# cyrillefavreau/Sol-R

Measured on AMD Instinct MI355X. Metric: Mrays/s @1920x1080, 3-bounce Cornell, higher is better.
Workload: dtype f32; 1 GPU; cornell 1920x1080, 3 bounces + shadow rays, 75 boxes / 29 primitives, one GPU, whole frame; rays_per_frame=6518779, closest_hit_walks_rank0=3506171, lane_nodes=206382796, lane_prim_tests=37557299, wave_nodes=3396811, wave_prim_tests=626627, wave_walks=106204, cost_ordered_launch_rank0=True, frames_in_flight=3, setup_frames_before_warmup=48, frames_delivered=9105, order_free_nodes=43, short_ray_lists=1, gather=none (one GPU), strips=equal rows, parallelism=tile1

## Files before the change

include/solr_hip.h:

```cpp
#ifndef SOLR_HIP_H
#define SOLR_HIP_H

#include "solr_types.h"

#ifdef __cplusplus
extern "C" {
#endif


void initialize_scene(vec2i occupancyParameters, SceneInfo sceneInfo, int nbPrimitives, int nbLamps,
                      int nbMaterials);

void finalize_scene(vec2i occupancyParameters);

void reshape_scene(vec2i occupancyParameters, SceneInfo sceneInfo);

void h2d_scene(vec2i occupancyParameters, BoundingBox *boundingBoxes, int nbActiveBoxes, Primitive *primitives,
               int nbPrimitives, Lamp *lamps, int nbLamps);

void h2d_materials(vec2i occupancyParameters, Material *materials, int nbActiveMaterials);

void h2d_randoms(vec2i occupancyParameters, float *randoms);

void h2d_textures(vec2i occupancyParameters, int activeTextures, TextureInfo *textureInfos);
// ... 55 lines not shown
int solr_hip_build_tree(const Primitive *primitives, const unsigned char *emissive, int nbPrimitives,
                        const float minPos[3], const float maxPos[3], float viewDistance, BoundingBox *boxes,
                        int boxCapacity, int *order, int *nbBoxes, int *nbLamps);
const char *solr_hip_build_tree_message(void);

void *solr_hip_device_bitmap(void);
void *solr_hip_device_primitive_ids(void);
void *solr_hip_device_postprocessing(void);
void solr_hip_bind_device_bitmap(void *deviceBitmap);

void solr_hip_h2d_randoms_sized(const float *randoms, long count);

int solr_hip_d2h_image_async(void);
const BitmapBuffer *solr_hip_image_wait(int ticket);
void solr_hip_set_copy_route(int onTheFramesOwnStream);
int solr_hip_stream_next_image(int on);
int solr_hip_d2h_streamed_image(BitmapBuffer *image);
int solr_hip_d2h_streamed(BitmapBuffer *image, PrimitiveXYIdBuffer *primitivesXYIds);
int solr_hip_image_share(const char *name, int rank, int world);
void solr_hip_image_share_sealed(void);
void solr_hip_image_unshare(void);

void solr_hip_d2h_postprocessing(PostProcessingBuffer *hostBuffer);
void solr_hip_h2d_postprocessing(const PostProcessingBuffer *hostBuffer, const PrimitiveXYIdBuffer *ids);

void solr_hip_initialize(const SceneInfo *sceneInfo);
void solr_hip_reshape(const SceneInfo *sceneInfo);
void solr_hip_render(const SceneInfo *sceneInfo, const vec4i *objects, const PostProcessingInfo *postProcessingInfo,
                     const float origin[3], const float direction[3], const float angles[4]);
void solr_hip_d2h(const SceneInfo *sceneInfo, BitmapBuffer *bitmap, PrimitiveXYIdBuffer *primitivesXYIds);

void solr_hip_enable_timing(int enable);
double solr_hip_kernel_time(int *nbLaunches, int reset);
int solr_hip_timing_samples(float *kernelMs, float *intervalMs, int capacity);

void solr_hip_set_frames_in_flight(int n);
int solr_hip_get_frames_in_flight(void);
void *solr_hip_flight_stream(int flight);
int solr_hip_next_flight(void);
void solr_hip_set_flight_streams(void *const *streams, int n);

void solr_hip_set_tile_scheduling(int mode);
int solr_hip_tile_scheduling_active(void);
int solr_hip_split_tiles(void);

void solr_hip_enable_tile_clocks(int enable);
int solr_hip_tile_clocks(unsigned long long *clocks, int capacityTiles);

void solr_hip_render_counting(const SceneInfo *sceneInfo, const vec4i *objects,
                              const PostProcessingInfo *postProcessingInfo, const float origin[3],
                              const float direction[3], const float angles[4], unsigned long long counts[8]);

void solr_hip_set_variant(int variant);
void solr_hip_set_short_ray_lists(int mode);
int solr_hip_short_ray_lists(void);
int solr_hip_order_free_nodes(void);
int solr_hip_order_free_shadows(void);
int solr_hip_get_variant(void);

void solr_hip_set_movable(const unsigned char *flags, int nbPrimitives);
int solr_hip_rotate_primitives(const float center[3], const float cosAngles[3], const float sinAngles[3],
                               float viewDistance);
int solr_hip_device_rotations(void);
int solr_hip_read_nodes(int exact, float *rows, int capacityRows);
int solr_hip_read_primitives(float *rows, int capacityRows);

void solr_hip_memory_usage(unsigned long long bytes[4]);

#ifdef __cplusplus
}
#endif
#endif
```

sol-r_amd/csrc/engine.h:

```cpp
#ifndef SOLR_ENGINE_H
#define SOLR_ENGINE_H

#include <hip/hip_runtime.h>

#include <atomic>
#include <chrono>
#include <cstdio>
#include <cstdlib>
#include <cstring>
#include <string>
#include <vector>

#include "../../include/solr_hip.h"
#include "renderer.h"
#include "lists_device.h"

namespace solreng
{
struct HostProfile
{
    const bool on = getenv("SOLR_HIP_HOST_PROFILE") != nullptr;
    struct Entry
    {
        const char *name;
// ... 63 lines not shown
struct DeviceBuffer
{
    void *ptr = nullptr;
    size_t bytes = 0;
};

const int MAX_FLIGHTS = 4;
struct SharedRing
{
    std::atomic<long> done[64][MAX_FLIGHTS + 2];
    std::atomic<long> consumed;
    long frameBytes, imageStride;
};
const int SORT_PERIOD = 64;

struct TileSchedule
{
    int mode = 1;
    DeviceBuffer cost, costSnapshot;
    DeviceBuffer order[2];
    int orderBuffer = 0;
    hipEvent_t orderEvent = nullptr;
    bool orderWait[MAX_FLIGHTS] = {};
    unsigned *hostStats = nullptr;
    unsigned *hostStatsDev = nullptr;
    long key[6] = {0, 0, 0, 0, 0, 0};
    int frames = 0;
    bool reorder = false;
    bool orderValid = false;
    BandCuts orderCuts = {};
    void reset()
    {
        frames = 0;
        reorder = false;
        orderValid = false;
    }
    void release();
};

enum Variant
{
    VARIANT_AUTOMATIC = 0,
    VARIANT_EXACT_LIST = 3,
    VARIANT_ALL_FEATURES = 4,
    VARIANT_NO_GROUPING = 5,
    VARIANT_NO_ORDER_FREE = 6,
    VARIANT_STACK_IN_LDS = 7,
    VARIANT_REFERENCE_LEAVES = 8,
    VARIANT_AO_FIXED_STRIDE = 9,
    VARIANT_NAN_DEEP_STACK = 10,
    VARIANT_UNSORTED_LISTS = 12,
    VARIANT_NO_BAND_WORDS = 13,
    VARIANT_ZERO_STREAM_COUNTERS = 14,
};

struct Engine
{
    bool initialized = false;
    int device = 0;
    hipStream_t stream = nullptr;
    bool ownStream = false;
    int errorCode = 0;
    std::string errorText;

    DeviceBuffer geometry, materials, textures, randoms, lamps;
    std::vector<float4> hostBoxes, hostBoxesCompact, hostPrims, hostLights;
    std::vector<int> hostBoxStart, hostBoxStartCompact, hostOriginCompact;
    int freeCountdown = 0;
    std::vector<float4> hostBoxesFree;
    std::vector<int> hostBoxStartFree;
    size_t freeRows = 0;
    bool freeHostValid = true;
    bool freeDirty = false;
    unsigned rowsFixed = 0;
    SolrDeviceLists freeStage;
    unsigned offBoxesFree = 0, offBoxStartFree = 0, offLeafFree = 0;
    int nbBoxesFree = 0;
    bool freeStale = false;
    bool primsContained = false;
    bool opaqueShadows = false;
    bool plainPlanes = false;
    float sceneExtent = 1.f;
    bool tightCompact = false, tightFree = false;
    bool sortedFree = false;
    int shortRayListsMode = -1;
    std::vector<int> materialTags;
    struct TextureUse
    {
        int material;
        long texels;
        long offsets[7];
    };
    std::vector<TextureUse> textureUses;
    size_t atlasBytes = 0;
    bool textureTablesChecked = false;
    std::vector<float> materialAverage;
    int sceneFeatures = F_ALL & ~F_FULL;
    unsigned offBoxes = 0, offBoxesCompact = 0, offBoxStart = 0, offBoxStartCompact = 0, offPrims = 0, offLights = 0;
    unsigned offLeaf = 0, offLeafCompact = 0;
    unsigned offMatCold = 0;
    bool geometryDirty = true;
    int nbBoxesCompact = 0;
    int orderedExact = 0, orderedCompact = 0;
    int nbBoxes = 0, nbPrimitives = 0, nbLights = 0, nbLamps = 0, nbMaterials = 0;
    int nested = 1;
    long nbRandoms = 0;

    DeviceBuffer pp, ids, bitmap, counters, tileClock;
    DeviceBuffer haloAbove[MAX_FLIGHTS], haloBelow[MAX_FLIGHTS], haloSendTop[MAX_FLIGHTS], haloSendBottom[MAX_FLIGHTS];
    DeviceBuffer haloGivenAbove, haloGivenBelow;
    int haloSuppliedAbove = 0, haloSuppliedBelow = 0;
    float randomsReach = 0.f;
    int haloWanted = -1;
    int flights = 1;
    hipStream_t extraStream[MAX_FLIGHTS - 1] = {};
    bool callerStreams = false;
    DeviceBuffer ppX[MAX_FLIGHTS - 1], idsX[MAX_FLIGHTS - 1], bitmapX[MAX_FLIGHTS - 1];
    int current = 0;
    unsigned frameSerial = 0;
    TileSchedule sched;
    unsigned lastSerial = 0;
    bool tileClocks = false;
    int nbTilesTimed = 0;
    void *boundBitmap = nullptr;
    int width = 0, height = 0;
    int firstRow = 0, nbRows = -1;
    int allocW = 0, allocRows = 0;

    int timing = 0;
    unsigned timingTick = 0;
    std::vector<std::pair<hipEvent_t, hipEvent_t>> events;
    double timedMs = 0.0;
    int timedLaunches = 0;
    std::vector<float> kernelSamples, intervalSamples;

    static const int IMAGE_RING = MAX_FLIGHTS + 2;
    hipStream_t copyStream = nullptr;
    BitmapBuffer *pinnedImage[IMAGE_RING] = {};
    size_t pinnedBytes = 0;
    hipEvent_t imageDone[IMAGE_RING] = {};
    hipEvent_t frameRendered = nullptr;
    static const long TICKET_PERIOD = ((long)0x7fffffff / IMAGE_RING / IMAGE_RING - 1) * IMAGE_RING;
    static int ticketOf(long serial, int slot) { return (int)((serial % TICKET_PERIOD) * IMAGE_RING + slot); }
    long imageSerial = 0;
    long slotSerial[IMAGE_RING] = {};
    long shareSeq = 0;
    long slotShareSeq[IMAGE_RING] = {};
    long lastWaitedSeq = 0;
    long sharePublished[IMAGE_RING] = {};
    struct SharedRing *sharedRing = nullptr;
    size_t sharedBytes = 0;
    std::string sharedName;
    int shareRank = 0, shareWorld = 0;
    bool slotOfStrips[IMAGE_RING] = {};
    long lastHandedOut = 0;
    bool copyOnRenderStream = false;
    int tileCheckedX = 0, tileCheckedTiles = 0, tileCheckedShift = 0;
    unsigned tileCheckedMagic = 0;
    DeviceBuffer bitmapAlt[MAX_FLIGHTS];
    DeviceBuffer deepStack[MAX_FLIGHTS];
    int bitmapSide[MAX_FLIGHTS] = {0, 0, 0, 0};
    int flightCopy[MAX_FLIGHTS][2] = {{-1, -1}, {-1, -1}, {-1, -1}, {-1, -1}};

    int streamNext = 0;
    bool streamedIds = false;
    bool streamedValid = false;
    const void *streamedBitmap = nullptr;
    unsigned streamSerial = 0;
    long streamKey[3] = {0, 0, 0};
    DeviceBuffer streamCounters;
    StreamPlan streamPlan = {};
    int streamBands = 0;
    unsigned *streamHostWords = nullptr;
// ... 252 lines not shown
```

sol-r_amd/csrc/renderer.h:

```cpp
#ifndef SOLR_RENDERER_H
#define SOLR_RENDERER_H

#include <hip/hip_runtime.h>

#include "../../include/solr_hip.h"
#include "rt_device.h"

using namespace solrdev;

struct FrameArgs
{
    SceneInfo si;
    PostProcessingInfo ppi;
    float ox, oy, oz;
    float dx, dy, dz;
    float ax, ay, az, aw;
    Trig trig;
    float stepx, stepy;
    int firstRow;
    int nbRows;
    int tilesX;
    unsigned tileMagic;
    int tileShift;
    int fuseDefault;
    int stackSlots;
    float4 *deepStack;
    long deepStride;
    float focusDepth;
    unsigned long long *tileClock;
    unsigned *tileCost;
    const unsigned *tileOrder;
    int nbTiles;
    unsigned *rowDone;
    const struct StreamPlan *streamPlan;
    unsigned streamSerial;
};

#define SOLR_STREAM_BANDS_MAX 8
struct StreamPlan
{
    unsigned *bandDone;
    unsigned *hostWord;
    int bands;
    int firstRow[SOLR_STREAM_BANDS_MAX + 1];
};

struct BandCuts
{
    int bands;
    int heavyShare;
    int firstTile[SOLR_STREAM_BANDS_MAX + 1];
};

#define ORDER_TILE_MASK 0x03ffffffu
#define ORDER_PART_SHIFT 26
#ifndef SOLR_SPLIT_LOG2
#define SOLR_SPLIT_LOG2 1
#endif
#define SPLIT_PARTS (1 << (2 * SOLR_SPLIT_LOG2))
#define ORDER_NOTHING 0xffffffffu
#define SOLR_TIMING_SLOTS (160000ul)
#define SPLIT_TILES_MAX 256

#ifndef SOLR_TILE_W_LOG2
#define SOLR_TILE_W_LOG2 3
#endif
#define TILE_W (1 << SOLR_TILE_W_LOG2)
#define TILE_H (64 >> SOLR_TILE_W_LOG2)
#define TILE 8
#define WAVE 64

struct PixelRecord
{
    float4 colorInfo;
    float4 sceneInfo;
};
static_assert(sizeof(PixelRecord) == sizeof(PostProcessingBuffer), "PixelRecord layout");


struct DepthHalo
{
    const float *above, *below;
    int nbAbove, nbBelow;
};

typedef void (*RendererFn)(const SceneArgs, const FrameArgs, PixelRecord *, int4 *, unsigned char *, unsigned long long *);
typedef void (*WalkBoundFn)(const SceneArgs, const char *, unsigned *, unsigned *);

namespace solrrows
// ... 41 lines not shown
```

sol-r_amd/csrc/renderer_kernel.h:

```cpp
#ifndef SOLR_RENDERER_KERNEL_H
#define SOLR_RENDERER_KERNEL_H

#include "renderer.h"

using namespace solrdev;

template <int COUNT, int FEAT, bool VOLUME = false>
#ifndef SOLR_GENERIC_WAVES
#define SOLR_GENERIC_WAVES 0
#endif
#ifndef SOLR_WAVES_PER_EU
#define SOLR_WAVES_PER_EU 4
#endif
__global__ __launch_bounds__(WAVE, (SOLR_GENERIC_WAVES && (FEAT & F_TEX)) ? SOLR_GENERIC_WAVES : SOLR_WAVES_PER_EU) void k_standardRenderer(const SceneArgs SA, const FrameArgs F,
                                                           PixelRecord *__restrict__ pp,
                                                           int4 *__restrict__ ids, unsigned char *__restrict__ bitmap,
                                                           unsigned long long *__restrict__ counters)
{
    extern __shared__ float ldsStack[];
    const Scene S = makeScene(SA);
    const SceneInfo &si = F.si;
    const int lane = threadIdx.x;
    const unsigned entry = F.tileOrder ? F.tileOrder[blockIdx.x] : blockIdx.x;
    if (entry == ORDER_NOTHING)
        return;
    const int tile = (int)min(entry & ORDER_TILE_MASK, (unsigned)F.nbTiles - 1u);
    const int part = (int)((entry >> ORDER_PART_SHIFT) & 31u);
    unsigned long long clock0 = 0ull;
    if (F.tileClock || F.tileCost)
        clock0 = __builtin_amdgcn_s_memrealtime();
    const int ty = F.tileMagic ? (int)(__umulhi((unsigned)tile, F.tileMagic) >> F.tileShift) : tile;
    const int tx = tile - ty * F.tilesX;
    const int x = tx * TILE_W + (lane & (TILE_W - 1));
    const int yLocal = ty * TILE_H + (lane >> SOLR_TILE_W_LOG2);
    const int W = si.size.x;
    const bool mine = part == 0 || ((((lane & (TILE_W - 1)) >> (SOLR_TILE_W_LOG2 - SOLR_SPLIT_LOG2)) |
                                     ((lane >> SOLR_TILE_W_LOG2) >> (6 - SOLR_TILE_W_LOG2 - SOLR_SPLIT_LOG2)) << SOLR_SPLIT_LOG2)) == part - 1;
#ifdef SOLR_PRIORITY_FOR_SPLIT_TILES
    if (part != 0)
        __builtin_amdgcn_s_setprio(SOLR_PRIORITY_FOR_SPLIT_TILES);
#endif
#ifdef SOLR_PRIORITY_FOR_FIRST_WAVES
    if (F.tileOrder && blockIdx.x < SOLR_PRIORITY_FOR_FIRST_WAVES)
        __builtin_amdgcn_s_setprio(2);
#endif
    const bool inside = mine && (x < W) && (yLocal < F.nbRows);
    const int index0 = inside ? yLocal * W + x : 0;
    const int yGlobal = F.firstRow + yLocal;
    const int gindex = yGlobal * W + x;

    constexpr bool volume = VOLUME;
    int4 id = make_int4(0, 0, 0, 0);
    bool active = inside;
    const bool refinementPass = si.pathTracingIteration > 0 && si.pathTracingIteration <= NB_MAX_ITERATIONS;
    if (inside && (refinementPass || volume))
    {
        id = ids[index0];
        if (refinementPass && si.pathTracingIteration > id.y && id.w == 0)
            active = false;
    }

    ColorStack cs;
    cs.base = ldsStack + lane;
    cs.stride = WAVE;
    cs.cold = 4 * F.stackSlots;
    cs.ldsSlots = F.stackSlots;
    cs.deep = (FEAT & F_STACK) ? F.deepStack + index0 : nullptr;
    cs.deepStride = F.deepStride;

    Counters cnt = {};
    if (COUNT == 2)
        cnt.record = (char *)counters + (size_t)blockIdx.x * SOLR_WALK_SLOT_BYTES;
    SOLR_T(const unsigned long long tKernel0 = SOLR_NOW();)

    v3 rayO = V(F.ox, F.oy, F.oz);
    v3 rayD = V(F.dx, F.dy, F.dz);
    v3 rotationCenter = V(0.f, 0.f, 0.f);
    if (si.cameraType == ctVR)
        rotationCenter = rayO;
    const bool antialiasingActivated = (FEAT & F_FULL) && (si.cameraType == ctAntialiazed);

    if (F.ppi.type != ppe_depthOfField && si.pathTracingIteration >= NB_MAX_ITERATIONS)
    {
        const float previousDepth = active ? pp[index0].colorInfo.w : 0.f;
        float a = (F.ppi.param1 / 20000.f);
        long rindex = (long)gindex + si.timestamp % (MAX_BITMAP_SIZE - 2);
        rayO.x += rnd(S, rindex) * previousDepth * a;
        rayO.y += rnd(S, rindex + 1) * previousDepth * a;
    }

    float dof = 0.f;
    if (si.cameraType == ctOrthographic)
    {
        rayD.x = rayO.z * 0.001f * (float)(x - (si.size.x / 2));
        rayD.y = -rayO.z * 0.001f * (float)(yGlobal - (si.size.y / 2));
        rayO.x = rayD.x;
        rayO.y = rayD.y;
    }
    else
    {
        rayD.x = rayD.x - F.stepx * (float)(x - (si.size.x / 2));
        rayD.y = rayD.y + F.stepy * (float)(yGlobal - (si.size.y / 2));
    }
    rayO = vectorRotation(rayO, rotationCenter, F.trig);
    rayD = vectorRotation(rayD, rotationCenter, F.trig);

    v3 color = V(0.f, 0.f, 0.f);
    if (!antialiasingActivated && (volume || si.pathTracingIteration >= NB_MAX_ITERATIONS))
    {
        const int k = si.pathTracingIteration % 4;
        rayD.x += (k == 0) ? 3.f : (k == 1) ? 5.f : (k == 2) ? -3.f : -5.f;
        rayD.y += (k == 0) ? 5.f : (k == 1) ? -3.f : (k == 2) ? -5.f : 3.f;
    }
    const bool anaglyph = (FEAT & F_FULL) && (si.cameraType == ctAnaglyph);
    const bool fishEye = (FEAT & F_FULL) && (si.cameraType == ctPanoramic);
    const bool vision = (FEAT & F_FULL) && (si.cameraType == ctVR);
    const bool plainStore = anaglyph || fishEye || vision;
    v3 leftEye = V(0.f, 0.f, 0.f);
    const int nbRays = antialiasingActivated ? 5 : (anaglyph ? 2 : 1);
#pragma unroll 1
    for (int I = 0; I < nbRays; ++I)
    {
        v3 rO = rayO;
        v3 rD = rayD;
        if (anaglyph)
// ... 170 lines not shown
        else
            ids[index] = id;

        if (F.fuseDefault)
        {
            v3 c = V(ppColor.x, ppColor.y, ppColor.z);
            if (si.pathTracingIteration > NB_MAX_ITERATIONS)
            {
                float d = (float)(si.pathTracingIteration - NB_MAX_ITERATIONS + 1);
                c.x /= d;
                c.y /= d;
                c.z /= d;
            }
            if ((FEAT & F_STREAM) && (F.fuseDefault & 2))
                makeColor<true>(si, c, bitmap, index);
            else
                makeColor(si, c, bitmap, index);
        }
    }
    if ((FEAT & F_STREAM) && (F.fuseDefault & 2))
    {
        asm volatile("s_waitcnt vmcnt(0)" ::: "memory");
        const unsigned units = partAgain ? 1u : (unsigned)SPLIT_PARTS;
        unsigned before = 0u;
        if (laneAgain == 0)
            before = __hip_atomic_fetch_add(F.rowDone + 64 * tyAgain, units, __ATOMIC_RELAXED, __HIP_MEMORY_SCOPE_AGENT);
        before = (unsigned)__builtin_amdgcn_readfirstlane((int)before);
        if (before + units == F.streamSerial * (unsigned)(F.tilesX * SPLIT_PARTS) && laneAgain == 0)
        {
            const StreamPlan *plan = F.streamPlan;
            int band = 0;
            while (band + 1 < plan->bands && tyAgain >= plan->firstRow[band + 1])
                ++band;
            const int rows = plan->firstRow[band + 1] - plan->firstRow[band];
            const unsigned rowsBefore = __hip_atomic_fetch_add(plan->bandDone + 64 * band, 1u, __ATOMIC_RELAXED, __HIP_MEMORY_SCOPE_AGENT);
            if (rowsBefore + 1u == F.streamSerial * (unsigned)rows)
                __hip_atomic_store(plan->hostWord + band, F.streamSerial, __ATOMIC_RELAXED, __HIP_MEMORY_SCOPE_SYSTEM);
        }
    }

    if (F.tileClock && laneAgain == 0)
    {
        F.tileClock[2 * tileAgain] = clock0;
        F.tileClock[2 * tileAgain + 1] = __builtin_amdgcn_s_memrealtime();
    }
    if (F.tileCost && laneAgain == 0)
    {
        const unsigned cost = (unsigned)(__builtin_amdgcn_s_memrealtime() - clock0);
        F.tileCost[tileAgain] = partAgain ? (unsigned)(SOLR_SPLIT_LOG2 + 1) * cost : cost;
    }
#ifdef SOLR_TIMING
    if (COUNT == 0 && laneAgain == 0 && counters)
    {
        unsigned long long *slot = counters + 16 + 16ull * blockIdx.x;
        slot[0] += SOLR_NOW() - tKernel0;
        slot[8] += cnt.tShade;
        slot[9] += cnt.tTrace;
        slot[10] += SOLR_NOW() - tEpilogue0;
        slot[1] += cnt.tClosest;
        slot[2] += cnt.tShadow;
        slot[3] += cnt.tNode;
        slot[4] += cnt.tLeaf;
        slot[5] += (unsigned long long)cnt.nAdvance;
        slot[6] += (unsigned long long)cnt.nLeaf;
        slot[7] += 1ull;
        slot[11] += cnt.tClosestPrimary;
        slot[12] += cnt.tAgain;
        slot[13] += ((unsigned long long)cnt.nAgain << 32) | cnt.nAgainLanes;
        slot[14] += ((unsigned long long)cnt.nAdvanceFirst << 32) | cnt.nAdvanceAgain;
        slot[15] += (unsigned long long)cnt.nChecked;
    }
#endif
    if (COUNT == 2 && lane == 0)
        ((int4 *)cnt.record)[0] = make_int4((int)cnt.ordinal, 0, 0, 0);
    if (COUNT == 1)
    {
        unsigned int vals[4] = {cnt.closest, cnt.shadow, cnt.boxes, cnt.prims};
#pragma unroll
        for (int k = 0; k < 4; ++k)
        {
            unsigned int v = vals[k];
            for (int off = 32; off > 0; off >>= 1)
                v += __shfl_xor(v, off, 64);
            if (lane == 0)
                atomicAdd(&counters[k], (unsigned long long)v);
        }
        if (lane == 0)
        {
            atomicAdd(&counters[4], (unsigned long long)cnt.wNodes);
            atomicAdd(&counters[5], (unsigned long long)cnt.wPrims);
            atomicAdd(&counters[6], (unsigned long long)cnt.wClosest);
            atomicAdd(&counters[7], (unsigned long long)cnt.wShadow);
        }
    }
}

template <int FEAT>
__global__ __launch_bounds__(WAVE, SOLR_WAVES_PER_EU) void k_walkBound(const SceneArgs SA, const char *__restrict__ records,
                                                                       unsigned *__restrict__ visits, unsigned *__restrict__ skipped)
{
    extern __shared__ float ldsStack[];
    const Scene S = makeScene(SA);
    const int lane = threadIdx.x;
    const char *slot = records + (size_t)blockIdx.x * SOLR_WALK_SLOT_BYTES;
    const int4 *head = (const int4 *)slot;
    const float4 *rays = (const float4 *)(slot + 16 * (SOLR_WALK_SLOTS + 1));
    const int recorded = __builtin_amdgcn_readfirstlane(head[0].x);
    const int walks = recorded < SOLR_WALK_SLOTS ? recorded : SOLR_WALK_SLOTS;
    unsigned entries = 0;
    int left_out = recorded - walks;
    for (int j = 0; j < walks; ++j)
    {
        const int4 h = head[1 + j];
        const int kind = __builtin_amdgcn_readfirstlane(h.x);
        if (kind == WALK_GENERAL)
        {
            ++left_out;
            continue;
        }
        const float4 a = rays[((size_t)j * 64 + lane) * 2], b = rays[((size_t)j * 64 + lane) * 2 + 1];
        const int doneAfter = __float_as_int(b.w);
        const bool took_part = doneAfter >= 0;
        const WalkRay r = makeWalkRay(V(a.x, a.y, a.z), took_part ? V(b.x, b.y, b.z) : V(1.f, 1.f, 1.f));
        Scene W = S;
        if (__builtin_amdgcn_readfirstlane(h.y))
        {
            const int octant = __builtin_amdgcn_readfirstlane(h.z);
            W.offBoxes = S.offBoxesFree + 2u * (unsigned)(octant * S.nbBoxesFree);
            W.offLeaf = S.offLeafFree + 4u * (unsigned)(octant * S.nbBoxesFree);
            W.nbBoxes = S.nbBoxesFree;
        }
        if (__builtin_amdgcn_readfirstlane(h.w) & 1)
            W.offBoxes += __builtin_amdgcn_readfirstlane(h.y) ? 16u * (unsigned)S.nbBoxesFree + 2u : 2u * (unsigned)S.nbBoxes + 2u;
        const int order = (FEAT & F_DEEP) ? (__builtin_amdgcn_readfirstlane(h.w) >> 1) & 3 : 0;
        if (order)
        {
            W.offBoxes += 32u * (unsigned)S.nbBoxesFree + 4u;
            W.nbBoxes = S.nbBoxesFree << 5;
        }
        const PackedRay pr = packRay(r);
        const float cutOff = a.w;
        int cursor = took_part ? 0 : SOLR_CURSOR_DONE;
        int cur = 0, visit = 0;
        while (cur < W.nbBoxes)
        {
// ... 26 lines not shown
```

sol-r_amd/csrc/solr_diag.hip:

```cpp
#include <hip/hip_runtime.h>
#include <dlfcn.h>
#include <fcntl.h>
#include <sched.h>
#include <sys/mman.h>
#include <sys/stat.h>
#include <unistd.h>

#include <atomic>

#include <cmath>
#include <cstdio>
#include <cstdlib>
#include <cstring>
#include <string>
#include <functional>
#include <chrono>
#include <vector>

#include "../../include/solr_hip.h"
#include "rt_device.h"
#include "device_pool.h"
#include "lists_device.h"

using namespace solrdev;
// ... 18 lines not shown
    *S = prepareScene(sceneInfo, exactNodes);
    if (!ok())
        return -1;
    *features = neededFeatures(sceneInfo, false);
    *deepList = deepNodeList(*S);
    *stream = flightStream(0);
    return 0;
}
void fail(int code, const char *what) { setError(code, what, __FILE__, __LINE__); }

int postProcess(const SceneInfo &sceneInfo, const PostProcessingInfo &ppInfo, const PostProcessingBuffer *frame,
                unsigned char *bitmapOut)
{
    if (!ready("solr_hip_probe_postprocess"))
        return -1;
    quiesce();
    HIPCHECK(hipSetDevice(g.device));
    ARGCHECK(frame != nullptr && bitmapOut != nullptr, "solr_hip_probe_postprocess: no buffer");
    ARGCHECK(sceneInfo.size.x > 0 && sceneInfo.size.y > 0, "solr_hip_probe_postprocess: empty image");
    ARGCHECK(g.nbRows < 0 && gDevices == 1, "solr_hip_probe_postprocess: whole frames of one device only");
    if (!ok())
        return -1;
    g.width = sceneInfo.size.x;
    g.height = sceneInfo.size.y;
    allocateFrame();
    if (!ok())
        return -1;
    const int flight = g.current;
    const hipStream_t stream = flightStream(flight);
    const size_t pixels = (size_t)g.width * g.height;
    HIPCHECK(hipMemcpyAsync(flightPp(flight).ptr, frame, pixels * sizeof(PostProcessingBuffer), hipMemcpyHostToDevice, stream));
    unsigned char *bitmap = (unsigned char *)flightBitmap(flight).ptr;
    const bool neighbourhood = (ppInfo.type == ppe_ambientOcclusion || ppInfo.type == ppe_depthOfField ||
                                ppInfo.type == ppe_radiosity || ppInfo.type == ppe_filter || ppInfo.type == ppe_cartoon);
    if (neighbourhood)
    {
        HaloDebt nothingOwed;
        launchPostProcess(sceneInfo, ppInfo, flight, stream, 0, g.height, bitmap, nothingOwed);
    }
    else
    {
        solrpost::defaultConversion(stream, sceneInfo, (int)pixels, (const PixelRecord *)flightPp(flight).ptr, bitmap);
        HIPCHECK(hipGetLastError());
    }
    HIPCHECK(hipMemcpyAsync(bitmapOut, bitmap, pixels * SOLR_COLOR_DEPTH, hipMemcpyDeviceToHost, stream));
    HIPCHECK(hipStreamSynchronize(stream));
    return ok() ? 0 : -1;
}

void lastFrame(int out[6])
{
    memcpy(out, g.lastFrame, sizeof(g.lastFrame));
}
}

extern "C" {
static unsigned long long walkLists[6];
void solr_hip_walk_bound_lists(unsigned long long out[6])
{
    if (out)
        memcpy(out, walkLists, sizeof(walkLists));
}

static int recordFrame(const SceneInfo *sceneInfo, const vec4i *objects, const PostProcessingInfo *postProcessingInfo,
                       const float origin[3], const float direction[3], const float angles[4], const char *who)
{
    quiesce();
    HIPCHECK(hipSetDevice(g.device));
    g.recorded = false;
    g.recordNext = true;
    if (!ok())
        return -1;
    renderImpl(*sceneInfo, *objects, *postProcessingInfo, origin, direction, angles, false, nullptr);
    g.recordNext = false;
    HIPCHECK(hipStreamSynchronize(flightStream(g.current)));
    if (!ok() || !g.recorded)
    {
        if (ok())
            setError(-1, "solr_hip_walk_bound: the frame was not recorded", __FILE__, __LINE__);
        return -1;
    }
    (void)who;
    return 0;
}

static int replayRecords(unsigned grid, size_t ldsBytes, int repeats, double ms[3], unsigned long long stats[4], bool lists)
{
    typedef WalkBoundFn BoundFn;
    ARGCHECK(g.recordVariant >= 0 && g.recordVariant < solrrows::LEAN_ROWS && g.walkRecords.ptr && grid > 0 &&
                 (size_t)grid * SOLR_WALK_SLOT_BYTES <= g.walkRecords.bytes,
             "solr_hip_walk_replay: no recorded frame, or more workgroups than its buffer holds");
    if (!ok())
        return -1;
    const BoundFn fn = solrrows::walkBound(g.recordVariant, solrrows::ROWS[g.recordVariant].features | (g.recordDeep ? F_DEEP : 0));
    ARGCHECK(fn != nullptr, "solr_hip_walk_bound: no replay instantiation for this row");
    if (!ok())
        return -1;
    reserve(g.walkVisits, (size_t)grid * WAVE * sizeof(unsigned) + 64);
    hipEvent_t e0 = nullptr, e1 = nullptr;
    HIPCHECK(hipEventCreate(&e0));
    HIPCHECK(hipEventCreate(&e1));
    if (!ok())
        return -1;
    const hipStream_t stream = flightStream(g.current);
    unsigned *visits = (unsigned *)g.walkVisits.ptr;
    unsigned *skipped = visits + (size_t)grid * WAVE;
    double sum = 0.0, best = 1.0e30;
    repeats = repeats < 1 ? 1 : repeats;
    for (int i = 0; i < repeats + 2 && ok(); ++i)
// ... 340 lines not shown
```

sol-r_amd/csrc/solr_hip.hip:

```cpp
#include <hip/hip_runtime.h>
#include <dlfcn.h>
#include <fcntl.h>
#include <sched.h>
#include <sys/mman.h>
#include <sys/stat.h>
#include <unistd.h>

#include <atomic>

#include <cmath>
#include <cstdio>
#include <cstdlib>
#include <cstring>
#include <string>
#include <functional>
#include <chrono>
#include <vector>

#include "../../include/solr_hip.h"
#include "rt_device.h"
#include "device_pool.h"
#include "lists_device.h"

using namespace solrdev;
// ... 180 lines not shown
    if (!g.stream)
    {
        HIPCHECK(hipStreamCreate(&g.stream));
        g.ownStream = ok();
        for (int f = 1; f < MAX_FLIGHTS && ok(); ++f)
            if (!g.extraStream[f - 1])
                HIPCHECK(hipStreamCreate(&g.extraStream[f - 1]));
    }
    g.initialized = ok();
    g.width = sceneInfo.size.x;
    g.height = sceneInfo.size.y;
}


static void finalizeOne()
{
    gHostProfile.report();
    if (!g.initialized)
        return;
    (void)hipSetDevice(g.device);
    if (g.stream)
        (void)hipStreamSynchronize(g.stream);
    for (hipStream_t extra : g.extraStream)
        if (extra)
            (void)hipStreamSynchronize(extra);
    collectEvents();
    DeviceBuffer *all[] = {&g.geometry, &g.materials, &g.textures, &g.randoms, &g.lamps,
                           &g.pp,       &g.ids,       &g.bitmap,   &g.counters, &g.tileClock,
                           &g.movable,  &g.refitPlan,
                           &g.walkRecords, &g.walkVisits};
    for (DeviceBuffer *b : all)
        release(*b);
    for (int f = 0; f < MAX_FLIGHTS; ++f)
    {
        release(g.deepStack[f]);
        release(g.haloAbove[f]);
        release(g.haloBelow[f]);
        release(g.haloSendTop[f]);
        release(g.haloSendBottom[f]);
    }
    release(g.haloGivenAbove);
    release(g.haloGivenBelow);
    g.haloSuppliedAbove = g.haloSuppliedBelow = 0;
    for (int f = 0; f < MAX_FLIGHTS - 1; ++f)
    {
        release(g.ppX[f]);
        release(g.idsX[f]);
        release(g.bitmapX[f]);
    }
    dropExtraStreams();
    releaseImageRing();
    releaseImageStreaming();
    g.sched.release();
    g.current = 0;
    if (g.ownStream && g.stream)
        (void)hipStreamDestroy(g.stream);
    g.stream = nullptr;
    g.ownStream = false;
    g.initialized = false;
    g.refitReady = false;
    g.refitPlanPending = false;
    g.hostOriginFree.clear();
    g.exactStale = false;
    g.deviceAhead = false;
    g.nbMovable = -1;
    g.nbDeviceRotations = 0;
    g.nbBoxes = g.nbPrimitives = g.nbLights = g.nbLamps = g.nbMaterials = 0;
    g.allocW = g.allocRows = 0;
    g.boundBitmap = nullptr;
    g.hostBoxes.clear();
    g.hostBoxesCompact.clear();
    g.hostPrims.clear();
    g.hostLights.clear();
    g.hostBoxStart.clear();
    g.hostBoxStartCompact.clear();
    g.hostBoxesFree.clear();
    g.hostBoxStartFree.clear();
    g.freeRows = 0;
    g.freeHostValid = true;
    g.freeDirty = false;
    dropFreeStage(true);
    {
        SolrScratchPool &pool = solrScratchPool();
        std::lock_guard<std::mutex> nobodyBuilding(pool.busy);
        pool.release();
    }
    g.hostOriginCompact.clear();
    g.nbBoxesFree = 0;
    g.freeCountdown = 0;
    g.freeStale = false;
    g.materialTags.clear();
    g.materialAverage.clear();
    g.geometryDirty = true;
}

static void reshapeOne(const SceneInfo &sceneInfo)
{
    if (!ready("reshape_scene"))
        return;
    quiesce();
    g.width = sceneInfo.size.x;
    g.height = sceneInfo.size.y;
    allocateFrame();
}


// ... 277 lines not shown
```

sol-r_amd/csrc/solr_launch.hip:

```cpp
#include <hip/hip_runtime.h>
#include <dlfcn.h>
#include <fcntl.h>
#include <sched.h>
#include <sys/mman.h>
#include <sys/stat.h>
#include <unistd.h>

#include <atomic>

#include <cmath>
#include <cstdio>
#include <cstdlib>
#include <cstring>
#include <string>
#include <functional>
#include <chrono>
#include <vector>

#include "../../include/solr_hip.h"
#include "rt_device.h"
#include "device_pool.h"
#include "lists_device.h"

using namespace solrdev;
// ... 490 lines not shown
static RendererFn recordingKernel(const KernelChoice &k, const SceneArgs &S, unsigned grid, size_t ldsBytes, hipStream_t stream)
{
    g.recordNext = false;
    ARGCHECK(k.row >= 0 && k.row < solrrows::LEAN_ROWS,
             "solr_hip_walk_bound: the kernel this scene needs has no recording instantiation (untextured spheres, "
             "planes, triangles, cylinders only)");
    if (!ok())
        return nullptr;
    reserve(g.walkRecords, (size_t)grid * SOLR_WALK_SLOT_BYTES);
    reserve(g.walkVisits, (size_t)grid * WAVE * sizeof(unsigned) + 64);
    if (!ok())
        return nullptr;
    HIPCHECK(hipMemsetAsync(g.walkRecords.ptr, 0, (size_t)grid * SOLR_WALK_SLOT_BYTES, stream));
    const RendererFn fn = solrrows::renderer(2, k.mask, false);
    ARGCHECK(fn != nullptr, "solr_hip_walk_bound: no recording instantiation");
    if (!ok())
        return nullptr;
    g.recordGrid = grid;
    g.recordLds = ldsBytes;
    g.recordDeep = (k.mask & F_DEEP) != 0;
    g.recordScene = S;
    g.recorded = true;
    return fn;
}

static bool armDeepStack(FrameArgs &F, int deepSlots, int flight, hipStream_t stream)
{
    F.stackSlots = SOLR_LDS_STACK_SLOTS;
    F.deepStride = (long)F.si.size.x * F.nbRows;
    reserve(g.deepStack[flight], (size_t)deepSlots * (size_t)F.deepStride * sizeof(float4));
    if (!ok())
        return false;
    F.deepStack = (float4 *)g.deepStack[flight].ptr;
    if (g.variant == VARIANT_NAN_DEEP_STACK)
        HIPCHECK(hipMemsetAsync(F.deepStack, 0xff, (size_t)deepSlots * (size_t)F.deepStride * sizeof(float4), stream));
    return true;
}

static bool armStreamedFrame(FrameArgs &F, const KernelChoice &k, const BandCuts &cuts, hipStream_t stream, bool withIds,
                             RendererFn *fn)
{
    if (k.mask < 0 || (F.tileOrder && memcmp(&g.sched.orderCuts, &cuts, sizeof(cuts)) != 0))
        return false;
    const RendererFn streaming = solrrows::renderer(0, k.mask | (k.deepSlots > 0 ? F_STACK : 0) | F_STREAM, false);
    if (!streaming || !armImageStreaming(F, tileRows(F), stream, withIds))
        return false;
    *fn = streaming;
    F.fuseDefault |= withIds ? 6 : 2;
    if (g.variant == VARIANT_NO_BAND_WORDS)
        F.streamSerial = 0x7fffff00u;
    return true;
}

void renderImpl(const SceneInfo &sceneInfo, const vec4i &objects, const PostProcessingInfo &ppInfo,
                const float origin[3], const float direction[3], const float angles[4], bool counting,
                unsigned long long counts[8])
{
    HostSpan whole("cudaRender (whole)");
    HaloDebt debt;
    if (ppInfo.type == ppe_ambientOcclusion && haveCommunicator())
    {
        debt.wanted = agreedHaloRows(ppInfo);
        debt.width = sceneInfo.size.x;
        debt.frameRows = sceneInfo.size.y;
        debt.owed = !(g.haloSuppliedAbove || g.haloSuppliedBelow);
    }
    if (!frameReady(sceneInfo, objects))
        return;
    const int flight = takeFlight(sceneInfo, counting);
    if (flight < 0)
        return;
    const hipStream_t stream = flightStream(flight);
    SceneArgs S;
    if (!frameScene(sceneInfo, objects, counting, S))
        return;
    FrameArgs F;
    if (!frameArgs(sceneInfo, ppInfo, origin, direction, angles, F))
        return;
    const unsigned tiles = (unsigned)(F.tilesX * tileRows(F));
    if (sceneInfo.cameraType == ctVR)
        readFocusDepth(F, flight, stream);
    if (g.tileClocks && !armTileClocks(F, tiles))
        return;
    bool streamIds = false;
    const BandCuts streamCuts = decideStreamCuts(F, counting, &streamIds);
    bool streamCandidate = streamCuts.bands > 0;
    if (g.sched.mode > 0 && !counting && !scheduleTiles(F, tiles, flight, stream, streamCuts, &streamCandidate))
        return;
    const std::pair<hipEvent_t, hipEvent_t> timer = startKernelTimer(counting, stream);

    const KernelChoice k = chooseKernel(sceneInfo, fullFeatures(sceneInfo), deepNodeList(S), counting);
    if (!counting)
        g.recordVariant = k.row;
    ARGCHECK(k.fn != nullptr, "cudaRender: no instantiation of the renderer for this scene (csrc/rows)");
    if (!ok())
        return;
    if (counting)
        HIPCHECK(hipMemsetAsync(g.counters.ptr, 0, 8 * sizeof(unsigned long long), stream));
    F.nbTiles = (int)tiles;
    const dim3 grid(F.tileOrder ? tiles + (unsigned)(SPLIT_PARTS - 1) * SPLIT_TILES_MAX : tiles);
    RendererFn fn = k.fn;
    const bool recording = g.recordNext && !counting;
    if (recording && !(fn = recordingKernel(k, S, grid.x, ldsBytesFor(F.stackSlots), stream)))
        return;
    unsigned long long *cntPtr = (unsigned long long *)(recording ? g.walkRecords.ptr : g.counters.ptr);
    if (k.deepSlots > 0 && !armDeepStack(F, k.deepSlots, flight, stream))
        return;
    unsigned char *bitmap = (unsigned char *)(g.boundBitmap ? g.boundBitmap : flightBitmap(flight).ptr);
    const bool streamed = streamCandidate && !recording && armStreamedFrame(F, k, streamCuts, stream, streamIds, &fn);
    g.lastMask = k.mask;
    g.streamedIds = streamed && streamIds;
    if (!counting)
    {
        const int features = k.mask < 0 ? -1 : k.mask | (k.deepSlots > 0 ? F_STACK : 0) | (streamed ? F_STREAM : 0);
        const int last[6] = {k.row, features, streamed ? 1 : 0, streamed ? streamCuts.bands : 0, F.tileOrder ? 1 : 0,
                             F.tileOrder ? g.sched.orderCuts.bands : 0};
        memcpy(g.lastFrame, last, sizeof(last));
    }
    {
        HostSpan launch("  of which the kernel launch");
        hipLaunchKernelGGL(fn, grid, dim3(WAVE), ldsBytesFor(F.stackSlots), stream, S, F, (PixelRecord *)flightPp(flight).ptr,
                           (int4 *)flightIds(flight).ptr, bitmap, cntPtr);
    }
    HIPCHECK(hipGetLastError());
    if (timer.first)
    {
        HIPCHECK(hipEventRecord(timer.second, stream));
        g.events.push_back(timer);
    }
    if (streamed)
    {
        markStreamedFrame(stream);
        g.streamedValid = ok();
        g.streamedBitmap = bitmap;
    }

    g.haloWanted = 0;
    if (neighbourhoodPass(ppInfo))
        launchPostProcess(sceneInfo, ppInfo, flight, stream, F.firstRow, F.nbRows, bitmap, debt);
    if (counting && counts)
    {
        HIPCHECK(hipMemcpyAsync(counts, g.counters.ptr, 8 * sizeof(unsigned long long), hipMemcpyDeviceToHost,
                                stream));
        HIPCHECK(hipStreamSynchronize(stream));
    }
}

void collectEvents()
{
    hipEvent_t before = nullptr;
    for (auto &ev : g.events)
    {
        float ms = 0.f, gap = 0.f;
        if (hipEventSynchronize(ev.second) == hipSuccess && hipEventElapsedTime(&ms, ev.first, ev.second) == hipSuccess)
        {
            g.timedMs += ms;
            g.timedLaunches++;
            if (g.kernelSamples.size() < 65536)
            {
                g.kernelSamples.push_back(ms);
                g.intervalSamples.push_back((before && hipEventElapsedTime(&gap, before, ev.second) == hipSuccess) ? gap : -1.f);
            }
        }
        if (before)
            (void)hipEventDestroy(before);
        (void)hipEventDestroy(ev.first);
        before = ev.second;
    }
    if (before)
        (void)hipEventDestroy(before);
    g.events.clear();
}
void d2hBitmapOne(const SceneInfo &sceneInfo, BitmapBuffer *bitmap, PrimitiveXYIdBuffer *primitivesXYIds, bool wait)
{
    if (!ready("d2h_bitmap"))
        return;
    HIPCHECK(hipSetDevice(g.device));
// ... 82 lines not shown
```

Baseline: 27280 Mrays/s.

## Replace one-workgroup-per-tile launch with persistent workgroups pulling tiles from atomic queue

The plain tile renderer now launches only as many workgroups as can be resident at once, and each one loops, taking tile entries from a per-flight atomic counter instead of using blockIdx. The host tracks a monotonically increasing queue base per flight, so the counter does not need resetting between frames. The goal is to remove workgroup dispatch overhead and tail imbalance across the cost-ordered tile list. The cost is one global atomic per tile and a loop around the inlined renderer, which may raise register pressure. It also depends on the occupancy query being correct.

```diff
diff --git a/include/solr_hip.h b/include/solr_hip.h
--- a/include/solr_hip.h
+++ b/include/solr_hip.h
@@ -131,6 +131,8 @@
                               const float direction[3], const float angles[4], unsigned long long counts[8]);
 
 void solr_hip_set_variant(int variant);
+void solr_hip_tile_queue_info(unsigned out[4]);
+int solr_hip_tile_queue_preset(unsigned value);
 void solr_hip_set_short_ray_lists(int mode);
 int solr_hip_short_ray_lists(void);
 int solr_hip_order_free_nodes(void);
diff --git a/sol-r_amd/csrc/engine.h b/sol-r_amd/csrc/engine.h
--- a/sol-r_amd/csrc/engine.h
+++ b/sol-r_amd/csrc/engine.h
@@ -139,6 +139,22 @@
     VARIANT_UNSORTED_LISTS = 12,
     VARIANT_NO_BAND_WORDS = 13,
     VARIANT_ZERO_STREAM_COUNTERS = 14,
+    VARIANT_WORKGROUP_PER_ENTRY = 15,
+};
+
+struct TileQueues
+{
+    DeviceBuffer words;
+    unsigned base[MAX_FLIGHTS] = {};
+    long key[3] = {0, 0, 0};
+    struct Resident
+    {
+        const void *fn;
+        size_t ldsBytes;
+        unsigned workgroups;
+    };
+    std::vector<Resident> resident;
+    unsigned last[4] = {0, 0, 0, 0};
 };
 
 struct Engine
@@ -206,6 +222,7 @@
     int current = 0;
     unsigned frameSerial = 0;
     TileSchedule sched;
+    TileQueues queues;
     unsigned lastSerial = 0;
     bool tileClocks = false;
     int nbTilesTimed = 0;
diff --git a/sol-r_amd/csrc/renderer.h b/sol-r_amd/csrc/renderer.h
--- a/sol-r_amd/csrc/renderer.h
+++ b/sol-r_amd/csrc/renderer.h
@@ -34,7 +34,18 @@
     unsigned *rowDone;
     const struct StreamPlan *streamPlan;
     unsigned streamSerial;
+    unsigned *tileQueue;
+    unsigned queueBase;
+    unsigned nbEntries;
 };
+
+namespace solrrows
+{
+constexpr bool drawsTiles(int count, int features, bool volume)
+{
+    return count == 0 && !volume && (features & (F_PROC | F_ELL | F_TEX | F_FULL | F_STREAM)) == 0;
+}
+}
 
 #define SOLR_STREAM_BANDS_MAX 8
 struct StreamPlan
diff --git a/sol-r_amd/csrc/renderer_kernel.h b/sol-r_amd/csrc/renderer_kernel.h
--- a/sol-r_amd/csrc/renderer_kernel.h
+++ b/sol-r_amd/csrc/renderer_kernel.h
@@ -5,23 +5,15 @@
 
 using namespace solrdev;
 
-template <int COUNT, int FEAT, bool VOLUME = false>
-#ifndef SOLR_GENERIC_WAVES
-#define SOLR_GENERIC_WAVES 0
-#endif
-#ifndef SOLR_WAVES_PER_EU
-#define SOLR_WAVES_PER_EU 4
-#endif
-__global__ __launch_bounds__(WAVE, (SOLR_GENERIC_WAVES && (FEAT & F_TEX)) ? SOLR_GENERIC_WAVES : SOLR_WAVES_PER_EU) void k_standardRenderer(const SceneArgs SA, const FrameArgs F,
-                                                           PixelRecord *__restrict__ pp,
-                                                           int4 *__restrict__ ids, unsigned char *__restrict__ bitmap,
-                                                           unsigned long long *__restrict__ counters)
+template <int COUNT, int FEAT, bool VOLUME>
+__device__ __forceinline__ void renderTile(const SceneArgs &SA, const FrameArgs &F, PixelRecord *__restrict__ pp,
+                                           int4 *__restrict__ ids, unsigned char *__restrict__ bitmap,
+                                           unsigned long long *__restrict__ counters, const unsigned slot, const int lane)
 {
     extern __shared__ float ldsStack[];
     const Scene S = makeScene(SA);
     const SceneInfo &si = F.si;
-    const int lane = threadIdx.x;
-    const unsigned entry = F.tileOrder ? F.tileOrder[blockIdx.x] : blockIdx.x;
+    const unsigned entry = F.tileOrder ? F.tileOrder[slot] : slot;
     if (entry == ORDER_NOTHING)
         return;
     const int tile = (int)min(entry & ORDER_TILE_MASK, (unsigned)F.nbTiles - 1u);
@@ -41,7 +33,7 @@
         __builtin_amdgcn_s_setprio(SOLR_PRIORITY_FOR_SPLIT_TILES);
 #endif
 #ifdef SOLR_PRIORITY_FOR_FIRST_WAVES
-    if (F.tileOrder && blockIdx.x < SOLR_PRIORITY_FOR_FIRST_WAVES)
+    if (F.tileOrder && slot < SOLR_PRIORITY_FOR_FIRST_WAVES)
         __builtin_amdgcn_s_setprio(2);
 #endif
     const bool inside = mine && (x < W) && (yLocal < F.nbRows);
@@ -70,7 +62,7 @@
 
     Counters cnt = {};
     if (COUNT == 2)
-        cnt.record = (char *)counters + (size_t)blockIdx.x * SOLR_WALK_SLOT_BYTES;
+        cnt.record = (char *)counters + (size_t)slot * SOLR_WALK_SLOT_BYTES;
     SOLR_T(const unsigned long long tKernel0 = SOLR_NOW();)
 
     v3 rayO = V(F.ox, F.oy, F.oz);
@@ -347,23 +339,23 @@
 #ifdef SOLR_TIMING
     if (COUNT == 0 && laneAgain == 0 && counters)
     {
-        unsigned long long *slot = counters + 16 + 16ull * blockIdx.x;
-        slot[0] += SOLR_NOW() - tKernel0;
-        slot[8] += cnt.tShade;
-        slot[9] += cnt.tTrace;
-        slot[10] += SOLR_NOW() - tEpilogue0;
-        slot[1] += cnt.tClosest;
-        slot[2] += cnt.tShadow;
-        slot[3] += cnt.tNode;
-        slot[4] += cnt.tLeaf;
-        slot[5] += (unsigned long long)cnt.nAdvance;
-        slot[6] += (unsigned long long)cnt.nLeaf;
-        slot[7] += 1ull;
-        slot[11] += cnt.tClosestPrimary;
-        slot[12] += cnt.tAgain;
-        slot[13] += ((unsigned long long)cnt.nAgain << 32) | cnt.nAgainLanes;
-        slot[14] += ((unsigned long long)cnt.nAdvanceFirst << 32) | cnt.nAdvanceAgain;
-        slot[15] += (unsigned long long)cnt.nChecked;
+        unsigned long long *sums = counters + 16 + 16ull * slot;
+        sums[0] += SOLR_NOW() - tKernel0;
+        sums[8] += cnt.tShade;
+        sums[9] += cnt.tTrace;
+        sums[10] += SOLR_NOW() - tEpilogue0;
+        sums[1] += cnt.tClosest;
+        sums[2] += cnt.tShadow;
+        sums[3] += cnt.tNode;
+        sums[4] += cnt.tLeaf;
+        sums[5] += (unsigned long long)cnt.nAdvance;
+        sums[6] += (unsigned long long)cnt.nLeaf;
+        sums[7] += 1ull;
+        sums[11] += cnt.tClosestPrimary;
+        sums[12] += cnt.tAgain;
+        sums[13] += ((unsigned long long)cnt.nAgain << 32) | cnt.nAgainLanes;
+        sums[14] += ((unsigned long long)cnt.nAdvanceFirst << 32) | cnt.nAdvanceAgain;
+        sums[15] += (unsigned long long)cnt.nChecked;
     }
 #endif
     if (COUNT == 2 && lane == 0)
@@ -386,6 +378,56 @@
             atomicAdd(&counters[5], (unsigned long long)cnt.wPrims);
             atomicAdd(&counters[6], (unsigned long long)cnt.wClosest);
             atomicAdd(&counters[7], (unsigned long long)cnt.wShadow);
+        }
+    }
+}
+
+struct RendererArgs
+{
+    SceneArgs SA;
+    FrameArgs F;
+    PixelRecord *pp;
+    int4 *ids;
+    unsigned char *bitmap;
+    unsigned long long *counters;
+};
+
+template <int COUNT, int FEAT, bool VOLUME = false>
+#ifndef SOLR_GENERIC_WAVES
+#define SOLR_GENERIC_WAVES 0
+#endif
+#ifndef SOLR_WAVES_PER_EU
+#define SOLR_WAVES_PER_EU 4
+#endif
+__global__ __launch_bounds__(WAVE, (SOLR_GENERIC_WAVES && (FEAT & F_TEX)) ? SOLR_GENERIC_WAVES : SOLR_WAVES_PER_EU) void k_standardRenderer(const SceneArgs SA, const FrameArgs F,
+                                                           PixelRecord *__restrict__ pp,
+                                                           int4 *__restrict__ ids, unsigned char *__restrict__ bitmap,
+                                                           unsigned long long *__restrict__ counters)
+{
+    if constexpr (!solrrows::drawsTiles(COUNT, FEAT, VOLUME))
+        renderTile<COUNT, FEAT, VOLUME>(SA, F, pp, ids, bitmap, counters, blockIdx.x, (int)threadIdx.x);
+    else
+    {
+        typedef const __attribute__((address_space(4))) RendererArgs *ArgumentSegment;
+        ArgumentSegment segment = (ArgumentSegment)__builtin_amdgcn_kernarg_segment_ptr();
+        unsigned slot = blockIdx.x;
+#pragma unroll 1
+        for (unsigned left = segment->F.tileQueue ? segment->F.nbEntries + 1u : 1u; left != 0u; --left)
+        {
+            asm volatile("" : "+s"(segment));
+            const RendererArgs &A = *(const RendererArgs *)segment;
+            int lane = (int)__builtin_amdgcn_mbcnt_hi(~0u, __builtin_amdgcn_mbcnt_lo(~0u, 0u));
+            asm volatile("" : "+v"(lane));
+            if (A.F.tileQueue)
+            {
+                unsigned ticket = 0u;
+                if (lane == 0)
+                    ticket = __hip_atomic_fetch_add(A.F.tileQueue, 1u, __ATOMIC_RELAXED, __HIP_MEMORY_SCOPE_AGENT);
+                slot = (unsigned)__builtin_amdgcn_readfirstlane((int)ticket) - A.F.queueBase;
+                if (slot >= A.F.nbEntries)
+                    break;
+            }
+            renderTile<COUNT, FEAT, VOLUME>(A.SA, A.F, A.pp, A.ids, A.bitmap, A.counters, slot, lane);
         }
     }
 }
diff --git a/sol-r_amd/csrc/solr_diag.hip b/sol-r_amd/csrc/solr_diag.hip
--- a/sol-r_amd/csrc/solr_diag.hip
+++ b/sol-r_amd/csrc/solr_diag.hip
@@ -94,9 +94,35 @@
 {
     memcpy(out, g.lastFrame, sizeof(g.lastFrame));
 }
+
 }
 
 extern "C" {
+void solr_hip_tile_queue_info(unsigned out[4])
+{
+    memcpy(out, g.queues.last, sizeof(g.queues.last));
+}
+
+int solr_hip_tile_queue_preset(unsigned value)
+{
+    if (!ready("solr_hip_tile_queue_preset"))
+        return -1;
+    TileQueues &q = g.queues;
+    if (!q.words.ptr)
+    {
+        reserve(q.words, (size_t)MAX_FLIGHTS * 64 * sizeof(unsigned));
+        if (ok())
+            HIPCHECK(hipMemset(q.words.ptr, 0, q.words.bytes));
+        memset(q.base, 0, sizeof(q.base));
+    }
+    for (int f = 0; f < MAX_FLIGHTS && ok(); ++f)
+        if (f == 0 || g.extraStream[f - 1])
+        {
+            HIPCHECK(hipMemsetD32Async((hipDeviceptr_t)((unsigned *)q.words.ptr + 64 * f), (int)value, 1, flightStream(f)));
+            q.base[f] = value;
+        }
+    return ok() ? 0 : -1;
+}
 static unsigned long long walkLists[6];
 void solr_hip_walk_bound_lists(unsigned long long out[6])
 {
diff --git a/sol-r_amd/csrc/solr_hip.hip b/sol-r_amd/csrc/solr_hip.hip
--- a/sol-r_amd/csrc/solr_hip.hip
+++ b/sol-r_amd/csrc/solr_hip.hip
@@ -256,6 +256,8 @@
     releaseImageRing();
     releaseImageStreaming();
     g.sched.release();
+    release(g.queues.words);
+    g.queues = TileQueues();
     g.current = 0;
     if (g.ownStream && g.stream)
         (void)hipStreamDestroy(g.stream);
diff --git a/sol-r_amd/csrc/solr_launch.hip b/sol-r_amd/csrc/solr_launch.hip
--- a/sol-r_amd/csrc/solr_launch.hip
+++ b/sol-r_amd/csrc/solr_launch.hip
@@ -566,6 +566,70 @@
     return true;
 }
 
+static unsigned residentWorkgroups(RendererFn fn, size_t ldsBytes)
+{
+    for (const TileQueues::Resident &r : g.queues.resident)
+        if (r.fn == (const void *)fn && r.ldsBytes == ldsBytes)
+            return r.workgroups;
+    int perCu = 0, cus = 0;
+    HIPCHECK(hipOccupancyMaxActiveBlocksPerMultiprocessor(&perCu, fn, WAVE, ldsBytes));
+    HIPCHECK(hipDeviceGetAttribute(&cus, hipDeviceAttributeMultiprocessorCount, g.device));
+    const unsigned workgroups = ok() && perCu > 0 && cus > 0 ? (unsigned)perCu * (unsigned)cus : 0u;
+    g.queues.resident.push_back({(const void *)fn, ldsBytes, workgroups});
+    return workgroups;
+}
+
+static unsigned armTileQueue(FrameArgs &F, RendererFn fn, bool draws, unsigned entries, size_t ldsBytes, int flight)
+{
+    TileQueues &q = g.queues;
+    memset(q.last, 0, sizeof(q.last));
+    if (!draws || g.variant == VARIANT_WORKGROUP_PER_ENTRY)
+        return entries;
+    const unsigned resident = residentWorkgroups(fn, ldsBytes);
+    if (resident == 0 || entries <= resident)
+        return entries;
+    const long key[3] = {(long)entries, F.si.size.x, F.nbRows};
+    if (!q.words.ptr || memcmp(key, q.key, sizeof(key)) != 0)
+    {
+        if (!q.words.ptr)
+        {
+            reserve(q.words, (size_t)MAX_FLIGHTS * 64 * sizeof(unsigned));
+            if (ok())
+                HIPCHECK(hipMemset(q.words.ptr, 0, q.words.bytes));
+            memset(q.base, 0, sizeof(q.base));
+        }
+        else
+            for (int f = 0; f < MAX_FLIGHTS; ++f)
+                if (f == 0 || g.extraStream[f - 1])
+                {
+                    HIPCHECK(hipMemsetAsync((unsigned *)q.words.ptr + 64 * f, 0, sizeof(unsigned), flightStream(f)));
+                    q.base[f] = 0;
+                }
+        if (!ok())
+            return entries;
+        memcpy(q.key, key, sizeof(key));
+    }
+    F.tileQueue = (unsigned *)q.words.ptr + 64 * flight;
+    F.queueBase = q.base[flight];
+    F.nbEntries = entries;
+    const unsigned last[4] = {resident, entries, q.base[flight], resident};
+    memcpy(q.last, last, sizeof(last));
+    return resident;
+}
+
+static void advanceTileQueue(const FrameArgs &F, unsigned workgroups, int flight, hipStream_t stream)
+{
+    if (!F.tileQueue)
+        return;
+    if (ok())
+        g.queues.base[flight] += F.nbEntries + workgroups;
+    else
+    {
+        (void)hipMemsetAsync(F.tileQueue, 0, sizeof(unsigned), stream);
+        g.queues.base[flight] = 0;
+    }
+}
+
 void renderImpl(const SceneInfo &sceneInfo, const vec4i &objects, const PostProcessingInfo &ppInfo,
                 const float origin[3], const float direction[3], const float angles[4], bool counting,
                 unsigned long long counts[8])
@@ -631,12 +695,18 @@
                              F.tileOrder ? g.sched.orderCuts.bands : 0};
         memcpy(g.lastFrame, last, sizeof(last));
     }
+    const bool draws = !counting && !recording && !streamed && k.mask >= 0 &&
+                       solrrows::drawsTiles(0, k.mask | (k.deepSlots > 0 ? F_STACK : 0), false);
+    const unsigned workgroups = armTileQueue(F, fn, draws, grid.x, ldsBytesFor(F.stackSlots), flight);
+    if (!ok())
+        return;
     {
         HostSpan launch("  of which the kernel launch");
-        hipLaunchKernelGGL(fn, grid, dim3(WAVE), ldsBytesFor(F.stackSlots), stream, S, F, (PixelRecord *)flightPp(flight).ptr,
-                           (int4 *)flightIds(flight).ptr, bitmap, cntPtr);
+        hipLaunchKernelGGL(fn, dim3(workgroups), dim3(WAVE), ldsBytesFor(F.stackSlots), stream, S, F,
+                           (PixelRecord *)flightPp(flight).ptr, (int4 *)flightIds(flight).ptr, bitmap, cntPtr);
     }
     HIPCHECK(hipGetLastError());
+    advanceTileQueue(F, workgroups, flight, stream);
     if (timer.first)
     {
         HIPCHECK(hipEventRecord(timer.second, stream));
```

Result: slower. 16580 Mrays/s (-39.2%).
